# hyperledger-labs/bdls

Measured on AMD Instinct MI355X. Metric: P-256 ECDSA verifies/sec (fused SHA-256, bit-exact vs Go crypto/ecdsa + Fabric low-S), higher is better.
Workload: dtype u32; 1 GPU; BASELINE config 2: 1048576 records/GPU, 256B messages, 65536 distinct keys, 1/16 corrupted, fused SHA-256; records_per_gpu=1048576, records_total=1048576, msg_len=256, nkeys=65536, corrupt_den=16, parallelism=shard1 (no collective)

## Files before the change

### bdls_amd/csrc/bdls_hip.cpp

```cpp
#include <hip/hip_runtime.h>

#include <algorithm>
#include <cctype>
#include <atomic>
#include <chrono>
#include <condition_variable>
#include <deque>
#include <memory>
#include <cstdio>
#include <cstdlib>
#include <cstring>
#include <functional>
#include <mutex>
#include <string>
#include <unordered_map>
#include <thread>
#include <vector>

#include "../../include/bdls_hip.h"
#include "verify.h"
#include "comb384.h"
#include "keys384.h"
#include "verify384.h"
#include "pack.h"
// ... 206 lines not shown
  bool defer = false;
  std::vector<std::vector<hipEvent_t>> ev_pool;
  size_t ev_used = 0;
  const uint32_t* last_counters = nullptr;
  uint32_t last_max_tables = 0, last_wide = 0;
  std::mutex mu;
};

std::mutex g_mu;
std::vector<Dev*> g_devs;

struct LaneRef {
  hipStream_t stream, aux;
  hipEvent_t fork, join, done, build;
  bool* done_recorded;
  DevBuf* ws;
};
LaneRef lane_ref(Dev& d, int l) {
  if (l <= 0) return LaneRef{d.stream, d.aux, d.fork, d.join, d.done, d.build, &d.done_recorded,
                             nullptr};
  Lane1& x = d.xl[l - 1];
  return LaneRef{x.stream, x.aux, x.fork, x.join, x.done, x.build, &x.done_recorded, &x.ws};
}

size_t max_tables_for(size_t ns, bool reg = false) {
  return std::min<size_t>(reg ? ns : ns / 2, size_t(1) << 16);
}

size_t qtab_slots(size_t ns) { return ns <= bh::kWide4Max ? 2 * ns : ns; }

size_t work_bytes(size_t ns) {
  const size_t hc = pow2_at_least(2 * ns);
  const size_t mt = max_tables_for(ns);
  return 4 * 32 * ns + 4 * 36 * ns + ns + qtab_slots(ns) * bh::kQTab * bh::kQPt * 4 +
         bh::kGPartWords * 4 * bh::gpart_slots(ns) +
         hc * (8 + 4 + 4 + 4) + ns * 16 + 16 + mt * 8 + mt * (size_t)bh::kKTabWords * 4 +
         256 * 27;
}

int carve_work(Dev& d, size_t n, bh::Work* w, bh::Plan* pl, bool reg = false,
               DevBuf* ws = nullptr) {
  const size_t ns = round64(n);
  DevBuf& buf = ws ? *ws : d.ws;
  int rc = buf.ensure(work_bytes(ns));
  if (rc) return rc;
  char* p = (char*)buf.p;
  auto take = [&](size_t bytes) {
    char* q = p;
    p += round256(bytes);
    return q;
  };
  w->ns = (uint32_t)ns;
  w->e = (uint32_t*)take(32 * ns);
  w->r = (uint32_t*)take(32 * ns);
  w->sm = (uint32_t*)take(32 * ns);
  w->pre = (uint32_t*)take(32 * ns);
  w->qx = (uint32_t*)take(36 * ns);
  w->qy = (uint32_t*)take(36 * ns);
  w->rm = (uint32_t*)take(36 * ns);
  w->r2m = (uint32_t*)take(36 * ns);
  w->st = (uint8_t*)take(ns);
  w->qtab = (uint32_t*)take(qtab_slots(ns) * bh::kQTab * bh::kQPt * 4);
  w->gpart = (uint32_t*)take(bh::kGPartWords * 4 * bh::gpart_slots(ns));
  const size_t hc = pow2_at_least(2 * ns);
  const size_t mt = max_tables_for(ns, reg);
  pl->hc = (uint32_t)hc;
  pl->max_tables = (uint32_t)mt;
  pl->slot_hash = (uint64_t*)take(hc * 8);
  pl->slot_rep = (uint32_t*)take(hc * 4);
  pl->slot_cnt = (uint32_t*)take(hc * 4);
  pl->slot_tab = (uint32_t*)take(hc * 4);
  pl->rec_slot = (uint32_t*)take(ns * 4);
  pl->comb_list = (uint32_t*)take(ns * 4);
  pl->comb_order = pl->comb_list;
  pl->ladder_list = (uint32_t*)take(ns * 4);
  pl->rec_tab = (uint32_t*)take(ns * 4);
  pl->counters = (uint32_t*)take(16);
  pl->tab_rec = (uint32_t*)take(mt * 4 + 4);
  pl->tab_dst = (uint32_t*)take(mt * 4 + 4);
  pl->tables = (uint32_t*)take(reg ? 4 : mt * (size_t)bh::kKTabWords * 4 + 4);
  return BH_OK;
}

hipError_t wait_lanes(Dev& d, hipStream_t s) {
  hipError_t e = hipSuccess;
  if (d.done_recorded && (e = hipStreamWaitEvent(s, d.done, 0)) != hipSuccess) return e;
  for (Lane1& x : d.xl)
    if (x.done_recorded && s != x.stream && (e = hipStreamWaitEvent(s, x.done, 0)) != hipSuccess)
      return e;
  return e;
}

int sync_lanes(Dev& d) {
// ... 2580 lines not shown
```

### bdls_amd/csrc/curve_consts.h

```cpp
#pragma once
#include <stdint.h>
namespace bh {
struct Fp_p256 {
  static constexpr uint32_t m[8] = {0xffffffffu, 0xffffffffu, 0xffffffffu, 0x00000000u, 0x00000000u, 0x00000000u, 0x00000001u, 0xffffffffu};
  static constexpr uint32_t n0 = 0x00000001u;
  static constexpr uint32_t r1[8] = {0x00000001u, 0x00000000u, 0x00000000u, 0xffffffffu, 0xffffffffu, 0xffffffffu, 0xfffffffeu, 0x00000000u};
  static constexpr uint32_t r2[8] = {0x00000003u, 0x00000000u, 0xffffffffu, 0xfffffffbu, 0xfffffffeu, 0xffffffffu, 0xfffffffdu, 0x00000004u};
  static constexpr uint32_t mm2[8] = {0xfffffffdu, 0xffffffffu, 0xffffffffu, 0x00000000u, 0x00000000u, 0x00000000u, 0x00000001u, 0xffffffffu};
  static constexpr uint32_t r3[8] = {0x0000000au, 0xfffffffdu, 0xfffffff7u, 0xffffffedu, 0xfffffffcu, 0x00000005u, 0x00000001u, 0x00000018u};
  static constexpr int32_t s30[9] = {1073741823, 1073741823, 1073741823, 63, 0, 0, 4096, 1073725440, 65535};
  static constexpr uint32_t inv30 = 0x3fffffffu;
};
struct Fn_p256 {
  static constexpr uint32_t m[8] = {0xfc632551u, 0xf3b9cac2u, 0xa7179e84u, 0xbce6faadu, 0xffffffffu, 0xffffffffu, 0x00000000u, 0xffffffffu};
  static constexpr uint32_t n0 = 0xee00bc4fu;
  static constexpr uint32_t r1[8] = {0x039cdaafu, 0x0c46353du, 0x58e8617bu, 0x43190552u, 0x00000000u, 0x00000000u, 0xffffffffu, 0x00000000u};
  static constexpr uint32_t r2[8] = {0xbe79eea2u, 0x83244c95u, 0x49bd6fa6u, 0x4699799cu, 0x2b6bec59u, 0x2845b239u, 0xf3d95620u, 0x66e12d94u};
  static constexpr uint32_t mm2[8] = {0xfc63254fu, 0xf3b9cac2u, 0xa7179e84u, 0xbce6faadu, 0xffffffffu, 0xffffffffu, 0x00000000u, 0xffffffffu};
  static constexpr uint32_t r3[8] = {0x0b65a624u, 0xac8ebec9u, 0x0c0555c9u, 0x111f28aeu, 0x6ba5e93fu, 0x2543b924u, 0x6407be65u, 0x503a54e7u};
  static constexpr int32_t s30[9] = {1013130577, 250030859, 830072911, 968797033, 1073741756, 1073741823, 4095, 1073725440, 65535};
  static constexpr uint32_t inv30 = 0x11ff43b1u;
};
struct Cv_p256 {
  static constexpr uint32_t b_m[8] = {0x29c4bddfu, 0xd89cdf62u, 0x78843090u, 0xacf005cdu, 0xf7212ed6u, 0xe5a220abu, 0x04874834u, 0xdc30061du};
  static constexpr uint32_t gx_m[8] = {0x18a9143cu, 0x79e730d4u, 0x5fedb601u, 0x75ba95fcu, 0x77622510u, 0x79fb732bu, 0xa53755c6u, 0x18905f76u};
  static constexpr uint32_t gy_m[8] = {0xce95560au, 0xddf25357u, 0xba19e45cu, 0x8b4ab8e4u, 0xdd21f325u, 0xd2e88688u, 0x25885d85u, 0x8571ff18u};
  static constexpr uint32_t half_n[8] = {0x7e3192a8u, 0x79dce561u, 0xd38bcf42u, 0xde737d56u, 0xffffffffu, 0x7fffffffu, 0x80000000u, 0x7fffffffu};
  static constexpr uint32_t p_minus_n[8] = {0x039cdaaeu, 0x0c46353du, 0x58e8617bu, 0x43190553u, 0x00000000u, 0x00000000u, 0x00000000u, 0x00000000u};
  static constexpr uint32_t n[8] = {0xfc632551u, 0xf3b9cac2u, 0xa7179e84u, 0xbce6faadu, 0xffffffffu, 0xffffffffu, 0x00000000u, 0xffffffffu};
  static constexpr uint32_t p[8] = {0xffffffffu, 0xffffffffu, 0xffffffffu, 0x00000000u, 0x00000000u, 0x00000000u, 0x00000001u, 0xffffffffu};
  static constexpr int a_is_minus3 = 1;
};
struct F30_p256 {
  static constexpr uint32_t p[9] = {0x3fffffffu, 0x3fffffffu, 0x3fffffffu, 0x0000003fu, 0x00000000u, 0x00000000u, 0x00001000u, 0x3fffc000u, 0x0000ffffu};
  static constexpr uint32_t n0 = 0x00000001u;
  static constexpr uint32_t r1[9] = {0x00004000u, 0x00000000u, 0x00000000u, 0x3ff00000u, 0x3fffffffu, 0x3fffffffu, 0x3bffffffu, 0x0fffffffu, 0x00000000u};
  static constexpr uint32_t r2[9] = {0x30000000u, 0x00000000u, 0x00000000u, 0x3ffffffcu, 0x3fffffbfu, 0x3fffffbfu, 0x3fffffffu, 0x3ffff7ffu, 0x00004fffu};
  static constexpr uint32_t r3[9] = {0x00006000u, 0x0000a000u, 0x3fff4000u, 0x3fdfffffu, 0x3fb7ffffu, 0x3fcfffffu, 0x3b7fffffu, 0x18ffffffu, 0x00000000u};
  using M32 = Fp_p256;
  static constexpr uint32_t k32[9] = {0x7fffffe0u, 0x7ffffffeu, 0x7ffffffeu, 0x400007feu, 0x3fffffffu, 0x3fffffffu, 0x4001ffffu, 0x7ff7ffffu, 0x001ffffeu};
  static constexpr uint32_t k64[9] = {0x7fffffc0u, 0x7ffffffeu, 0x7ffffffeu, 0x40000ffeu, 0x3fffffffu, 0x3fffffffu, 0x4003ffffu, 0x7fefffffu, 0x003ffffeu};
  static constexpr uint32_t b_m[9] = {0x2f77f70cu, 0x1f6229c4u, 0x02436273u, 0x1cc9c543u, 0x35ab3c01u, 0x2bf7212eu, 0x1025c882u, 0x1e0b7483u, 0x00000187u};
  static constexpr uint32_t gx_m[9] = {0x050f0624u, 0x30d418a9u, 0x1805e79cu, 0x1fc475dbu, 0x041d6ea5u, 0x2b776225u, 0x1985adccu, 0x2bdc755cu, 0x000017ddu};
  static constexpr uint32_t gy_m[9] = {0x1582a15cu, 0x1357ce95u, 0x117377c9u, 0x0e434a9eu, 0x0962d2aeu, 0x08dd21f3u, 0x1535e21au, 0x0aaf85d8u, 0x00007fc6u};
  static constexpr uint32_t pm2[8] = {0xfffffffdu, 0xffffffffu, 0xffffffffu, 0x00000000u, 0x00000000u, 0x00000000u, 0x00000001u, 0xffffffffu};
  static constexpr int a_is_minus3 = 1;
  static constexpr int sparse_p256 = 1;
};
struct Fp_k1 {
  static constexpr uint32_t m[8] = {0xfffffc2fu, 0xfffffffeu, 0xffffffffu, 0xffffffffu, 0xffffffffu, 0xffffffffu, 0xffffffffu, 0xffffffffu};
  static constexpr uint32_t n0 = 0xd2253531u;
  static constexpr uint32_t r1[8] = {0x000003d1u, 0x00000001u, 0x00000000u, 0x00000000u, 0x00000000u, 0x00000000u, 0x00000000u, 0x00000000u};
  static constexpr uint32_t r2[8] = {0x000e90a1u, 0x000007a2u, 0x00000001u, 0x00000000u, 0x00000000u, 0x00000000u, 0x00000000u, 0x00000000u};
  static constexpr uint32_t mm2[8] = {0xfffffc2du, 0xfffffffeu, 0xffffffffu, 0xffffffffu, 0xffffffffu, 0xffffffffu, 0xffffffffu, 0xffffffffu};
  static constexpr uint32_t r3[8] = {0x3795f671u, 0x002bb1e3u, 0x00000b73u, 0x00000001u, 0x00000000u, 0x00000000u, 0x00000000u, 0x00000000u};
  static constexpr int32_t s30[9] = {1073740847, 1073741819, 1073741823, 1073741823, 1073741823, 1073741823, 1073741823, 1073741823, 65535};
  static constexpr uint32_t inv30 = 0x2ddacacfu;
};
struct Fn_k1 {
  static constexpr uint32_t m[8] = {0xd0364141u, 0xbfd25e8cu, 0xaf48a03bu, 0xbaaedce6u, 0xfffffffeu, 0xffffffffu, 0xffffffffu, 0xffffffffu};
  static constexpr uint32_t n0 = 0x5588b13fu;
  static constexpr uint32_t r1[8] = {0x2fc9bebfu, 0x402da173u, 0x50b75fc4u, 0x45512319u, 0x00000001u, 0x00000000u, 0x00000000u, 0x00000000u};
  static constexpr uint32_t r2[8] = {0x67d7d140u, 0x896cf214u, 0x0e7cf878u, 0x741496c2u, 0x5bcd07c6u, 0xe697f5e4u, 0x81c69bc5u, 0x9d671cd5u};
  static constexpr uint32_t mm2[8] = {0xd036413fu, 0xbfd25e8cu, 0xaf48a03bu, 0xbaaedce6u, 0xfffffffeu, 0xffffffffu, 0xffffffffu, 0xffffffffu};
  static constexpr uint32_t r3[8] = {0xe9ff41edu, 0x7bc0cfe0u, 0x44d4322cu, 0x00176484u, 0xf1d0b2dau, 0xb1b31347u, 0x18ef116du, 0x555d800cu};
  static constexpr int32_t s30[9] = {271991105, 1061780019, 881460155, 733428139, 1073741498, 1073741823, 1073741823, 1073741823, 65535};
  static constexpr uint32_t inv30 = 0x2a774ec1u;
};
struct Cv_k1 {
  static constexpr uint32_t b_m[8] = {0x00001ab7u, 0x00000007u, 0x00000000u, 0x00000000u, 0x00000000u, 0x00000000u, 0x00000000u, 0x00000000u};
  static constexpr uint32_t gx_m[8] = {0x487e2097u, 0xd7362e5au, 0x29bc66dbu, 0x231e2953u, 0x33fd129cu, 0x979f48c0u, 0xe9089f48u, 0x9981e643u};
  static constexpr uint32_t gy_m[8] = {0xd3dbabe2u, 0xb15ea6d2u, 0x1f1dc64du, 0x8dfc5d5du, 0xac19c136u, 0x70b6b59au, 0xd4a582d6u, 0xcf3f851fu};
  static constexpr uint32_t half_n[8] = {0x681b20a0u, 0xdfe92f46u, 0x57a4501du, 0x5d576e73u, 0xffffffffu, 0xffffffffu, 0xffffffffu, 0x7fffffffu};
  static constexpr uint32_t p_minus_n[8] = {0x2fc9baeeu, 0x402da172u, 0x50b75fc4u, 0x45512319u, 0x00000001u, 0x00000000u, 0x00000000u, 0x00000000u};
  static constexpr uint32_t n[8] = {0xd0364141u, 0xbfd25e8cu, 0xaf48a03bu, 0xbaaedce6u, 0xfffffffeu, 0xffffffffu, 0xffffffffu, 0xffffffffu};
  static constexpr uint32_t p[8] = {0xfffffc2fu, 0xfffffffeu, 0xffffffffu, 0xffffffffu, 0xffffffffu, 0xffffffffu, 0xffffffffu, 0xffffffffu};
  static constexpr int a_is_minus3 = 0;
};
struct F30_k1 {
  static constexpr uint32_t p[9] = {0x3ffffc2fu, 0x3ffffffbu, 0x3fffffffu, 0x3fffffffu, 0x3fffffffu, 0x3fffffffu, 0x3fffffffu, 0x3fffffffu, 0x0000ffffu};
  static constexpr uint32_t n0 = 0x12253531u;
  static constexpr uint32_t r1[9] = {0x00f44000u, 0x00010000u, 0x00000000u, 0x00000000u, 0x00000000u, 0x00000000u, 0x00000000u, 0x00000000u, 0x00000000u};
  static constexpr uint32_t r2[9] = {0x10000000u, 0x0003a428u, 0x000007a2u, 0x00000004u, 0x00000000u, 0x00000000u, 0x00000000u, 0x00000000u, 0x00000000u};
  static constexpr uint32_t r3[9] = {0x00000000u, 0x1f671000u, 0x2c78cde5u, 0x0b73002bu, 0x00040000u, 0x00000000u, 0x00000000u, 0x00000000u, 0x00000000u};
  using M32 = Fp_k1;
  static constexpr uint32_t k32[9] = {0x7fff85e0u, 0x7fffff7eu, 0x7ffffffeu, 0x7ffffffeu, 0x7ffffffeu, 0x7ffffffeu, 0x7ffffffeu, 0x7ffffffeu, 0x001ffffeu};
  static constexpr uint32_t k64[9] = {0x7fff0bc0u, 0x7ffffefeu, 0x7ffffffeu, 0x7ffffffeu, 0x7ffffffeu, 0x7ffffffeu, 0x7ffffffeu, 0x7ffffffeu, 0x003ffffeu};
  static constexpr uint32_t b_m[9] = {0x06adc000u, 0x00070000u, 0x00000000u, 0x00000000u, 0x00000000u, 0x00000000u, 0x00000000u, 0x00000000u, 0x00000000u};
  static constexpr uint32_t gx_m[9] = {0x08b83460u, 0x2e5ae1feu, 0x1b6f5cd8u, 0x15329bc6u, 0x2708c78au, 0x0033fd12u, 0x225e7d23u, 0x3e9089f4u, 0x00007990u};
  static constexpr uint32_t gy_m[9] = {0x2bbe38ffu, 0x26d3a317u, 0x1936c57au, 0x15d1f1dcu, 0x0da37f17u, 0x1aac19c1u, 0x19c2dad6u, 0x3d4a582du, 0x0000e147u};
  static constexpr uint32_t pm2[8] = {0xfffffc2du, 0xfffffffeu, 0xffffffffu, 0xffffffffu, 0xffffffffu, 0xffffffffu, 0xffffffffu, 0xffffffffu};
  static constexpr int a_is_minus3 = 0;
  static constexpr int sparse_p256 = 0;
};
}
```

### bdls_amd/csrc/fp30.h

```cpp
#pragma once
#include "bh_common.h"
#include "curve_consts.h"

#ifndef BH_ZFILTER
#define BH_ZFILTER 0
#endif

namespace bh {

constexpr uint32_t kM30 = 0x3fffffffu;
constexpr int kL = 9;

BH_HD void f_copy(uint32_t r[9], const uint32_t a[9]) {
#pragma unroll
  for (int i = 0; i < 9; i++) r[i] = a[i];
}

BH_HD void f_sel(uint32_t r[9], bool c, const uint32_t a[9], const uint32_t b[9]) {
#pragma unroll
  for (int i = 0; i < 9; i++) r[i] = c ? a[i] : b[i];
}

template <class C>
BH_HD void f_const(uint32_t r[9], const C& c) {
// ... 27 lines not shown
    }
#pragma unroll
    for (int k = 8; k < 17; k++) {
      acc += C[k];
      const uint32_t m = (uint32_t)acc & kM30;
      if (k == 8) {
        mac_k<64u>(C[11], m);
        mac_k<4096u>(C[14], m);
        mac_k<F::p[7]>(C[15], m);
        mac_k<F::p[8]>(C[16], m);
      } else {
        r[k - 9] = m;
      }
      acc >>= 30;
    }
  } else {
#pragma unroll
    for (int k = 0; k < 17; k++) {
      acc += C[k];
      if (k < 9) {
        const uint32_t m = ((uint32_t)acc * F::n0) & kM30;
        acc += (uint64_t)m * F::p[0];
#pragma unroll
        for (int j = 1; j < 9; j++)
          if (F::p[j]) C[k + j] += (uint64_t)m * F::p[j];
      } else {
        r[k - 9] = (uint32_t)acc & kM30;
      }
      acc >>= 30;
    }
  }
  r[8] = (uint32_t)acc;
}

template <class F>
BH_HD void f_mul(uint32_t r[9], const uint32_t a[9], const uint32_t b[9]) {
  uint64_t C[17];
#pragma unroll
  for (int k = 0; k < 17; k++) C[k] = 0;
#pragma unroll
  for (int i = 0; i < 9; i++)
#pragma unroll
    for (int j = 0; j < 9; j++) C[i + j] += (uint64_t)a[i] * b[j];
  f_redc<F>(r, C);
}

template <class F>
BH_HD void f_sqr(uint32_t r[9], const uint32_t a[9]) {
  uint64_t C[17];
  uint32_t d[9];
#pragma unroll
  for (int i = 0; i < 9; i++) d[i] = a[i] << 1;
#pragma unroll
  for (int k = 0; k < 17; k++) C[k] = 0;
#pragma unroll
  for (int i = 0; i < 9; i++) {
    C[2 * i] += (uint64_t)a[i] * a[i];
#pragma unroll
    for (int j = i + 1; j < 9; j++) C[i + j] += (uint64_t)d[i] * a[j];
  }
  f_redc<F>(r, C);
}

BH_HD void f_add(uint32_t r[9], const uint32_t a[9], const uint32_t b[9]) {
  uint32_t c = 0;
#pragma unroll
// ... 298 lines not shown
```

### bdls_amd/csrc/gen_consts.py

```python
#!/usr/bin/env python3
import sys

CURVES = {
    "p256": dict(
        p=2**256 - 2**224 + 2**192 + 2**96 - 1,
        n=0xFFFFFFFF00000000FFFFFFFFFFFFFFFFBCE6FAADA7179E84F3B9CAC2FC632551,
        a=-3,
        b=0x5AC635D8AA3A93E7B3EBBD55769886BC651D06B0CC53B0F63BCE3C3E27D2604B,
        gx=0x6B17D1F2E12C4247F8BCE6E563A440F277037D812DEB33A0F4A13945D898C296,
        gy=0x4FE342E2FE1A7F9B8EE7EB4A7C0F9E162BCE33576B315ECECBB6406837BF51F5,
    ),
    "k1": dict(
        p=2**256 - 2**32 - 977,
        n=0xFFFFFFFFFFFFFFFFFFFFFFFFFFFFFFFEBAAEDCE6AF48A03BBFD25E8CD0364141,
        a=0,
        b=7,
        gx=0x79BE667EF9DCBBAC55A06295CE870B07029BFCDB2DCE28D959F2815B16F81798,
        gy=0x483ADA7726A3C4655DA4FBFC0E1108A8FD17B448A68554199C47D08FFB10D4B8,
    ),
}
R = 2**256


def limbs(v):
# ... 8 lines not shown
    print(f"  static constexpr uint32_t r1[8] = {{{limbs(R % m)}}};  // R mod m")
    print(f"  static constexpr uint32_t r2[8] = {{{limbs(R * R % m)}}};  // R^2 mod m")
    print(f"  static constexpr uint32_t mm2[8] = {{{limbs(m - 2)}}};  // m - 2 (Fermat exponent)")
    print(f"  static constexpr uint32_t r3[8] = {{{limbs(R * R * R % m)}}};  // R^3 mod m")
    s30 = ", ".join(f"{(m >> (30 * i)) & ((1 << 30) - 1) if i < 8 else m >> 240}" for i in range(9))
    print(f"  static constexpr int32_t s30[9] = {{{s30}}};  // m in signed radix 2^30")
    print(f"  static constexpr uint32_t inv30 = 0x{pow(m, -1, 2**30):08x}u;  // m^-1 mod 2^30")
    print("};")


W = 30
MASK = (1 << W) - 1
R30 = 2**270


def limbs30(v):
    assert 0 <= v < 2**300
    out = [(v >> (W * i)) & MASK for i in range(9)]
    out[8] = v >> (W * 8)
    assert out[8] < 2**32
    return ", ".join(f"0x{x:08x}u" for x in out)


def borrowed30(v):
    l = [(v >> (W * i)) & MASK for i in range(9)]
    l[8] = v >> (W * 8)
    for i in range(8):
        l[i] += 1 << W
        l[i + 1] -= 1
    assert sum(x << (W * i) for i, x in enumerate(l)) == v and min(l) >= 0
    return ", ".join(f"0x{x:08x}u" for x in l)


def emit_fp30(name, c):
    p = c["p"]
    n0 = (-pow(p, -1, 2**W)) % 2**W
    print(f"struct {name} {{  // radix 2^30, R = 2^270")
    print(f"  static constexpr uint32_t p[9] = {{{limbs30(p)}}};")
    print(f"  static constexpr uint32_t n0 = 0x{n0:08x}u;  // -p^-1 mod 2^30")
    print(f"  static constexpr uint32_t r1[9] = {{{limbs30(R30 % p)}}};  // R mod p")
    print(f"  static constexpr uint32_t r2[9] = {{{limbs30(R30 * R30 % p)}}};  // R^2 mod p")
    print(f"  static constexpr uint32_t r3[9] = {{{limbs30(R30 ** 3 % p)}}};  // R^3 mod p (safegcd inverse)")
    print(f"  using M32 = Fp_{name[4:]};  // the same field on 32-bit limbs (fe.h safegcd)")
    print(f"  static constexpr uint32_t k32[9] = {{{borrowed30(32 * p)}}};  // 32p, borrowed form")
    print(f"  static constexpr uint32_t k64[9] = {{{borrowed30(64 * p)}}};  // 64p, borrowed form")
    print(f"  static constexpr uint32_t b_m[9] = {{{limbs30(c['b'] * R30 % p)}}};  // b R mod p")
    print(f"  static constexpr uint32_t gx_m[9] = {{{limbs30(c['gx'] * R30 % p)}}};")
    print(f"  static constexpr uint32_t gy_m[9] = {{{limbs30(c['gy'] * R30 % p)}}};")
    print(f"  static constexpr uint32_t pm2[8] = {{{limbs(p - 2)}}};  // Fermat exponent (32-bit limbs)")
    print(f"  static constexpr int a_is_minus3 = {1 if c['a'] == -3 else 0};")
    print(f"  static constexpr int sparse_p256 = {1 if p == 2**256 - 2**224 + 2**192 + 2**96 - 1 else 0};")
    print("};")


def main():
    print("// GENERATED by gen_consts.py -- do not edit.")
    print("#pragma once")
    print("#include <stdint.h>")
    print("namespace bh {")
    for cname, c in CURVES.items():
        emit_mod(f"Fp_{cname}", c["p"])
        emit_mod(f"Fn_{cname}", c["n"])
        p = c["p"]
        print(f"struct Cv_{cname} {{")
        print(f"  static constexpr uint32_t b_m[8] = {{{limbs(c['b'] * R % p)}}};  // b*R mod p")
        print(f"  static constexpr uint32_t gx_m[8] = {{{limbs(c['gx'] * R % p)}}};")
        print(f"  static constexpr uint32_t gy_m[8] = {{{limbs(c['gy'] * R % p)}}};")
        print(f"  static constexpr uint32_t half_n[8] = {{{limbs(c['n'] >> 1)}}};  // floor(n/2)")
        print(f"  static constexpr uint32_t p_minus_n[8] = {{{limbs(p - c['n'])}}};  // p - n")
        print(f"  static constexpr uint32_t n[8] = {{{limbs(c['n'])}}};")
        print(f"  static constexpr uint32_t p[8] = {{{limbs(p)}}};")
        print(f"  static constexpr int a_is_minus3 = {1 if c['a'] == -3 else 0};")
        print("};")
        emit_fp30(f"F30_{cname}", c)
    print("}  // namespace bh")


P384 = dict(
    p=2**384 - 2**128 - 2**96 + 2**32 - 1,
    n=0xFFFFFFFFFFFFFFFFFFFFFFFFFFFFFFFFFFFFFFFFFFFFFFFFC7634D81F4372DDF581A0DB248B0A77AECEC196ACCC52973,
    a=-3,
    b=0xB3312FA7E23EE7E4988E056BE3F82D19181D9C6EFE8141120314088F5013875AC656398D8A2ED19D2A85C8EDD3EC2AEF,
    gx=0xAA87CA22BE8B05378EB1C71EF320AD746E1D3B628BA79B9859F741E082542A385502F25DBF55296C3A545E3872760AB7,
    gy=0x3617DE4A96262C6F5D9E98BF9292DC29F8F41DBD289A147CE9DA3113B5F0B8C00A60B1CE1D7E819D7A431D7C90EA0E5F,
)
W28 = 28
L28 = 14
R28 = 2**(W28 * L28)
KP_MAX = 32


def limbs28(v):
    assert 0 <= v < R28
    return ", ".join(f"0x{(v >> (W28 * i)) & (2**W28 - 1):07x}u" for i in range(L28))


def words12(v):
    assert 0 <= v < 2**384
    return ", ".join(f"0x{(v >> (32 * i)) & 0xffffffff:08x}u" for i in range(12))


def emit_mod28(name, m):
    n0 = (-pow(m, -1, 2**W28)) % 2**W28
    print(f"struct {name} {{  // radix 2^28, 14 limbs, R = 2^392")
    print(f"  static constexpr uint32_t m[14] = {{{limbs28(m)}}};")
    print(f"  static constexpr uint32_t n0 = 0x{n0:07x}u;  // -m^-1 mod 2^28")
# ... 35 lines not shown
```

### bdls_amd/csrc/verify.h

```cpp
#pragma once
#include <type_traits>

#include "blake2b.h"
#include "der.h"
#include "fe.h"
#include "ec30.h"
#include "sha256.h"
#include "sha3.h"

namespace bh {

enum : uint32_t {
  BHF_HASH_SHA256 = 1u,
  BHF_NO_LOW_S = 2u,
  BHF_HASH_SHA3_256 = 8u,
  BHF_BDLS_PREHASHED = 0x100u,
};

enum : int { HK_GIVEN_OR_SHA256 = 0, HK_SHA3_256 = 1 };

enum : uint8_t { ST_R2OK = 0x80u };

struct BatchIn {
  const uint8_t* pub;
// ... 97 lines not shown
};

#ifndef BH_AOS
#define BH_AOS 1
#endif
BH_HD void ld8(uint32_t v[8], const uint32_t* base, uint32_t i, uint32_t ns) {
#if BH_AOS
  const W4* p = reinterpret_cast<const W4*>(base + (size_t)i * 8);
  const W4 a = p[0], b = p[1];
  v[0] = a.x; v[1] = a.y; v[2] = a.z; v[3] = a.w;
  v[4] = b.x; v[5] = b.y; v[6] = b.z; v[7] = b.w;
#else
#pragma unroll
  for (int k = 0; k < 8; k++) v[k] = base[(size_t)k * ns + i];
#endif
}
BH_HD void st8(uint32_t* base, uint32_t i, uint32_t ns, const uint32_t v[8]) {
#if BH_AOS
  W4* p = reinterpret_cast<W4*>(base + (size_t)i * 8);
  p[0] = W4{v[0], v[1], v[2], v[3]};
  p[1] = W4{v[4], v[5], v[6], v[7]};
#else
#pragma unroll
  for (int k = 0; k < 8; k++) base[(size_t)k * ns + i] = v[k];
#endif
}
BH_HD void ld9(uint32_t v[9], const uint32_t* base, uint32_t i, uint32_t ns) {
#pragma unroll
  for (int k = 0; k < 9; k++) v[k] = BH_AOS ? base[(size_t)i * 9 + k] : base[(size_t)k * ns + i];
}
BH_HD void st9(uint32_t* base, uint32_t i, uint32_t ns, const uint32_t v[9]) {
#pragma unroll
  for (int k = 0; k < 9; k++) (BH_AOS ? base[(size_t)i * 9 + k] : base[(size_t)k * ns + i]) = v[k];
}

template <class P, class C>
BH_HD bool key_import(const uint8_t* q, uint32_t qx30[9], uint32_t qy30[9]) {
  uint32_t qx[8], qy[8], pp[8];
  load_const8(pp, C::p);
  be32_to_limbs(qx, q);
  be32_to_limbs(qy, q + 32);
  if (geq8(qx, pp) || geq8(qy, pp)) return false;
  f_from_u256(qx30, qx);
  f_from_u256(qy30, qy);
  f_to_mont<P>(qx30, qx30);
  f_to_mont<P>(qy30, qy30);
  f_canon<P>(qx30, qx30);
  f_canon<P>(qy30, qy30);
  return j_on_curve<P>(qx30, qy30);
}

template <class P, class C>
BH_HD void stage_prep_key(const BatchIn& in, const Work& w, uint32_t i) {
  uint32_t qx30[9], qy30[9];
  const bool ok = key_import<P, C>(in.pub + (size_t)i * 64, qx30, qy30);
  if (!ok) {
    f_const(qx30, P::gx_m);
    f_const(qy30, P::gy_m);
  }
  st9(w.qx, i, w.ns, qx30);
  st9(w.qy, i, w.ns, qy30);
  w.st[i] = ok ? (uint8_t)R_OK : (uint8_t)R_BAD_KEY;
}

template <class C, int HK>
BH_HD void digest_e(const BatchIn& in, uint32_t i, uint32_t e[8]) {
// ... 26 lines not shown
  uint32_t nn[8], t[8];
  load_const8(nn, C::n);
  const uint32_t bo = sub8(t, e, nn);
  if (!bo) copy8(e, t);
}

template <class P, class N, class C, int HK = HK_GIVEN_OR_SHA256, bool DEFER = false>
BH_HD void stage_prep(const BatchIn& in, const Work& w, uint32_t i) {
  uint8_t reason = R_OK;
  uint32_t r[8], s[8], e[8];
  uint32_t qx30[9], qy30[9];
  const uint32_t slen = in.sig_len[i];
  const uint32_t mlen = in.msg_len[i];
  const bool fused = HK == HK_SHA3_256 || (in.flags & BHF_HASH_SHA256) != 0;
  if (slen == 0) reason = R_EMPTY_SIG;
  else if (!fused && mlen == 0) reason = R_EMPTY_DIGEST;
  DerSig ds;
  if (reason == R_OK) reason = der_parse_sig(in.sig + in.sig_off[i], slen, &ds);
  uint32_t half[8], nn[8];
  load_const8(half, C::half_n);
  load_const8(nn, C::n);
  if (reason == R_OK) {
    copy8(r, ds.r);
    copy8(s, ds.s);
    if (!(in.flags & BHF_NO_LOW_S) && (ds.s_big || !geq8(half, s))) reason = R_HIGH_S;
  }
  if (reason == R_OK && !key_import<P, C>(in.pub + (size_t)i * 64, qx30, qy30))
    reason = R_BAD_KEY;
  if (reason == R_OK && (ds.r_big || geq8(r, nn))) reason = R_R_RANGE;
  if (reason == R_OK && (ds.s_big || geq8(s, nn))) reason = R_S_RANGE;
  if (reason == R_OK && !DEFER) digest_e<C, HK>(in, i, e);
  uint8_t st = reason;
  if (reason == R_OK) {
    uint32_t pmn[8], rn[8], rm[9], r2m[9];
    load_const8(pmn, C::p_minus_n);
    f_from_u256(rm, r);
    f_to_mont<P>(rm, rm);
    f_canon<P>(rm, rm);
    if (!geq8(r, pmn)) {
      st |= ST_R2OK;
      add8(rn, r, nn);
      f_from_u256(r2m, rn);
      f_to_mont<P>(r2m, r2m);
      f_canon<P>(r2m, r2m);
    } else {
      f_copy(r2m, rm);
    }
    st9(w.rm, i, w.ns, rm);
    st9(w.r2m, i, w.ns, r2m);
    to_mont<N>(s, s);
  } else {
    for (int k = 0; k < 8; k++) { e[k] = r[k] = 0; }
    e[0] = r[0] = 1;
    load_const8(s, N::r1);
    f_const(qx30, P::gx_m);
    f_const(qy30, P::gy_m);
  }
  if (!DEFER) st8(w.e, i, w.ns, e);
  st8(w.r, i, w.ns, r);
  st8(w.sm, i, w.ns, s);
  st9(w.qx, i, w.ns, qx30);
  st9(w.qy, i, w.ns, qy30);
  w.st[i] = st;
}

BH_HD void setbytes_u256(const uint8_t* b, uint32_t len, uint32_t v[8], bool* big, bool* zero) {
  uint32_t lo = 0;
  while (lo < len && b[lo] == 0) lo++;
  const uint32_t L = len - lo;
  *zero = (L == 0);
  *big = (L > 32);
#pragma unroll
  for (int k = 0; k < 8; k++) v[k] = 0;
  if (L > 32) return;
#pragma unroll
  for (int j = 0; j < 32; j++) {
    uint32_t x = 0;
    if ((uint32_t)j < L) x = b[len - 1 - j];
    v[j >> 2] |= x << (8 * (j & 3));
  }
}

template <class C>
BH_HD void stage_bdls_given(const BdlsIn& in, const Work& w, uint32_t i) {
  uint32_t e[8], nn[8], t[8];
  const uint8_t* m = in.msg + in.msg_off[i];
  const uint32_t mlen = in.msg_len[i];
// ... 13 lines not shown

template <class C>
BH_HD void stage_bdls_hash(const BdlsIn& in, const Work& w, uint32_t i) {
  if (in.flags & BHF_BDLS_PREHASHED) return stage_bdls_given<C>(in, w, i);
  uint8_t hsh[32];
  uint32_t e[8], nn[8], t[8];
  const uint8_t* q = in.xy + (size_t)i * 64;
  bdls_signed_proto_hash(hsh, in.version[i], q, q + 32, in.msg + in.msg_off[i], in.msg_len[i]);
  be32_to_limbs(e, hsh);
  load_const8(nn, C::n);
  if (!sub8(t, e, nn)) copy8(e, t);
  st8(w.e, i, w.ns, e);
}

template <class P, class N, class C>
BH_HD void stage_prep(const BdlsIn& in, const Work& w, uint32_t i) {
  uint8_t reason = R_OK;
  uint32_t r[8], s[8], nn[8];
  uint32_t qx30[9], qy30[9];
  load_const8(nn, C::n);
  bool rbig, rzero, sbig, szero;
  setbytes_u256(in.r + in.r_off[i], in.r_len[i], r, &rbig, &rzero);
  setbytes_u256(in.s + in.s_off[i], in.s_len[i], s, &sbig, &szero);
  if (rzero) reason = R_R_NONPOS;
  else if (szero) reason = R_S_NONPOS;
  const uint8_t* q = in.xy + (size_t)i * 64;
  const bool badkey = reason == R_OK && !key_import<P, C>(q, qx30, qy30);
  if (badkey && P::a_is_minus3) reason = R_BAD_KEY;
  if (reason == R_OK && (rbig || geq8(r, nn))) reason = R_R_RANGE;
  if (reason == R_OK && (sbig || geq8(s, nn))) reason = R_S_RANGE;
  if (reason == R_OK && badkey) reason = R_MATH;
  uint8_t st = reason;
  if (reason == R_OK) {
    uint32_t pmn[8], rn[8], rm[9], r2m[9];
    load_const8(pmn, C::p_minus_n);
    f_from_u256(rm, r);
    f_to_mont<P>(rm, rm);
    f_canon<P>(rm, rm);
    if (!geq8(r, pmn)) {
      st |= ST_R2OK;
      add8(rn, r, nn);
      f_from_u256(r2m, rn);
      f_to_mont<P>(r2m, r2m);
      f_canon<P>(r2m, r2m);
    } else {
      f_copy(r2m, rm);
    }
    st9(w.rm, i, w.ns, rm);
    st9(w.r2m, i, w.ns, r2m);
    to_mont<N>(s, s);
  } else {
    for (int k = 0; k < 8; k++) r[k] = 0;
    r[0] = 1;
    load_const8(s, N::r1);
    f_const(qx30, P::gx_m);
    f_const(qy30, P::gy_m);
  }
  st8(w.r, i, w.ns, r);
  st8(w.sm, i, w.ns, s);
  st9(w.qx, i, w.ns, qx30);
  st9(w.qy, i, w.ns, qy30);
  w.st[i] = st;
}

template <class N, bool U1 = true, bool VAR = false>
BH_HD void stage_inv(const Work& w, uint32_t c, uint32_t stride, uint32_t n) {
  uint32_t acc[8], x[8];
  load_const8(acc, N::r1);
  uint32_t last = c;
  for (uint32_t i = c; i < n; i += stride) {
    st8(w.pre, i, w.ns, acc);
    ld8(x, w.sm, i, w.ns);
    mont_mul<N>(acc, acc, x);
    last = i;
  }
  if (c >= n) return;
  uint32_t inv[8];
  mont_inv_sg<N, VAR>(inv, acc);
  for (uint32_t i = last;; i -= stride) {
    uint32_t pre[8], wi[8], t[8];
    ld8(pre, w.pre, i, w.ns);
    mont_mul<N>(wi, inv, pre);
    ld8(x, w.sm, i, w.ns);
    mont_mul<N>(inv, inv, x);
    if constexpr (U1) {
      ld8(t, w.e, i, w.ns);
      mont_mul<N>(t, t, wi);
      st8(w.e, i, w.ns, t);
    } else {
      st8(w.sm, i, w.ns, wi);
    }
    ld8(t, w.r, i, w.ns);
    mont_mul<N>(t, t, wi);
    st8(w.r, i, w.ns, t);
    if (i < c + stride) break;
  }
}

template <class N>
BH_HD void calc_u1(uint32_t u1[8], const Work& w, uint32_t i) {
  uint32_t wi[8];
  ld8(u1, w.e, i, w.ns);
  ld8(wi, w.sm, i, w.ns);
  mont_mul<N>(u1, u1, wi);
}

BH_HD void booth5(uint32_t in6, uint32_t* mag, bool* neg) {
  uint32_t sgn = 0u - (in6 >> 5);
  uint32_t d = (63u - in6) & sgn;
  d |= in6 & ~sgn;
  *mag = (d >> 1) + (d & 1u);
  *neg = sgn != 0;
}


BH_HD uint32_t* qtab_entry(uint32_t* tab, uint32_t wave, uint32_t entry, uint32_t lane) {
  return tab + (((size_t)wave * 64 + lane) * kQTab + entry) * kQPt;
}

BH_HD void qtab_store(uint32_t* tab, uint32_t wave, uint32_t entry, uint32_t lane, const J30& P) {
  uint32_t v[28];
#pragma unroll
  for (int k = 0; k < 9; k++) {
    v[k] = P.X[k];
    v[9 + k] = P.Y[k];
    v[18 + k] = P.Z[k];
  }
  v[27] = 0;
  W4* d = reinterpret_cast<W4*>(qtab_entry(tab, wave, entry, lane));
#pragma unroll
  for (int q = 0; q < 7; q++) d[q] = W4{v[4 * q], v[4 * q + 1], v[4 * q + 2], v[4 * q + 3]};
}

BH_HD void qtab_load(J30& P, const uint32_t* tab, uint32_t wave, uint32_t entry, uint32_t lane) {
  const W4* s = reinterpret_cast<const W4*>(qtab_entry(const_cast<uint32_t*>(tab), wave, entry, lane));
  uint32_t v[28];
#pragma unroll
// ... 155 lines not shown
      mag = nmag;
      neg = nneg;
    } else {
      g_window(v, win, gtab, tx, ty, mag, neg);
      if (neg) f_neg<P, 64>(ty, ty);
      g_step<P>(B, b_inf, tx, ty, mag, one);
    }
  }
}

template <class P>
BH_HD bool finish_check(const Work& w, uint32_t i, const J30& A, bool a_inf, const J30& B,
                        bool b_inf) {
  J30 Pt;
  bool p_inf;
  if (b_inf) {
    j_copy(Pt, A);
    p_inf = a_inf;
  } else if (a_inf) {
    j_copy(Pt, B);
    p_inf = false;
  } else {
    bool same;
    const bool deg = j_add<P>(Pt, A, B, &same);
    p_inf = false;
    if (deg) {
      if (same) j_dbl<P>(Pt, A);
      else p_inf = true;
    }
  }
  uint32_t z2[9], t[9], x[9], rm[9];
  f_sqr<P>(z2, Pt.Z);
  const bool z_zero = f_is_zero2<P>(z2);
  f_reduce<P>(x, Pt.X);
  ld9(rm, w.rm, i, w.ns);
  f_mul<P>(t, rm, z2);
  f_canon<P>(t, t);
  bool ok = f_eq(t, x);
  if (w.st[i] & ST_R2OK) {
    ld9(rm, w.r2m, i, w.ns);
    f_mul<P>(t, rm, z2);
    f_canon<P>(t, t);
    ok = ok || f_eq(t, x);
  }
  return ok && !p_inf && !z_zero;
}

template <class P>
BH_HD void q_ladder(J30& A, bool& a_inf, const Work& w, uint32_t i, uint32_t wave,
                    uint32_t lane) {
  uint32_t u2[8], qx[9], qy[9], one[9];
  ld8(u2, w.r, i, w.ns);
  ld9(qx, w.qx, i, w.ns);
  ld9(qy, w.qy, i, w.ns);
  f_const(one, P::r1);
  J30 T;
  f_copy(T.X, qx);
  f_copy(T.Y, qy);
  f_copy(T.Z, one);
  qtab_store(w.qtab, wave, 0, lane, T);
  j_dbl<P>(T, T);
  qtab_store(w.qtab, wave, 1, lane, T);
  for (uint32_t k = 2; k < kQTab; k++) {
    bool same;
    j_madd<P>(T, T, qx, qy, &same);
    qtab_store(w.qtab, wave, k, lane, T);
  }
  uint32_t K[9];
  K[0] = u2[0] << 28;
#pragma unroll
  for (int k = 1; k < 8; k++) K[k] = (u2[k] << 28) | (u2[k - 1] >> 4);
  K[8] = u2[7] >> 4;
  {
    uint32_t mag;
    bool neg;
    booth5(K[8] >> 26, &mag, &neg);
// ... 1360 lines not shown
```

Before: 209.3 million verifies/s.

## Move scalar arithmetic onto the radix-2^30 multiplier and drop stored r+n candidate

```diff
diff --git a/bdls_amd/csrc/bdls_hip.cpp b/bdls_amd/csrc/bdls_hip.cpp
--- a/bdls_amd/csrc/bdls_hip.cpp
+++ b/bdls_amd/csrc/bdls_hip.cpp
@@ -262,7 +262,7 @@
 size_t work_bytes(size_t ns) {
   const size_t hc = pow2_at_least(2 * ns);
   const size_t mt = max_tables_for(ns);
-  return 4 * 32 * ns + 4 * 36 * ns + ns + qtab_slots(ns) * bh::kQTab * bh::kQPt * 4 +
+  return 4 * 32 * ns + 3 * 36 * ns + ns + qtab_slots(ns) * bh::kQTab * bh::kQPt * 4 +
          bh::kGPartWords * 4 * bh::gpart_slots(ns) +
          hc * (8 + 4 + 4 + 4) + ns * 16 + 16 + mt * 8 + mt * (size_t)bh::kKTabWords * 4 +
          256 * 27;
@@ -288,7 +288,7 @@
   w->qx = (uint32_t*)take(36 * ns);
   w->qy = (uint32_t*)take(36 * ns);
   w->rm = (uint32_t*)take(36 * ns);
-  w->r2m = (uint32_t*)take(36 * ns);
+  w->r2m = nullptr;
   w->st = (uint8_t*)take(ns);
   w->qtab = (uint32_t*)take(qtab_slots(ns) * bh::kQTab * bh::kQPt * 4);
   w->gpart = (uint32_t*)take(bh::kGPartWords * 4 * bh::gpart_slots(ns));
diff --git a/bdls_amd/csrc/curve_consts.h b/bdls_amd/csrc/curve_consts.h
--- a/bdls_amd/csrc/curve_consts.h
+++ b/bdls_amd/csrc/curve_consts.h
@@ -1,6 +1,7 @@
 #pragma once
 #include <stdint.h>
 namespace bh {
+template <class M> struct Scalar30;
 struct Fp_p256 {
   static constexpr uint32_t m[8] = {0xffffffffu, 0xffffffffu, 0xffffffffu, 0x00000000u, 0x00000000u, 0x00000000u, 0x00000001u, 0xffffffffu};
   static constexpr uint32_t n0 = 0x00000001u;
@@ -31,6 +32,16 @@
   static constexpr uint32_t p[8] = {0xffffffffu, 0xffffffffu, 0xffffffffu, 0x00000000u, 0x00000000u, 0x00000000u, 0x00000001u, 0xffffffffu};
   static constexpr int a_is_minus3 = 1;
 };
+struct N30_p256 {
+  static constexpr uint32_t p[9] = {0x3c632551u, 0x0ee72b0bu, 0x3179e84fu, 0x39beab69u, 0x3fffffbcu, 0x3fffffffu, 0x00000fffu, 0x3fffc000u, 0x0000ffffu};
+  static constexpr uint32_t n0 = 0x2e00bc4fu;
+  static constexpr uint32_t r1[9] = {0x36abc000u, 0x353d039cu, 0x05ec3118u, 0x15258e86u, 0x0010c641u, 0x00000000u, 0x3c000000u, 0x0fffffffu, 0x00000000u};
+  static constexpr uint32_t r2[9] = {0x0887ac57u, 0x05d911a5u, 0x130785e0u, 0x2a328ab8u, 0x19076a9eu, 0x1afb1658u, 0x2484a92bu, 0x2a0ebf05u, 0x000055abu};
+  static constexpr uint32_t r3[9] = {0x2fc38adfu, 0x3fa3e2bbu, 0x1b018b23u, 0x095feb0bu, 0x110fb41du, 0x13f26264u, 0x0f2dd97au, 0x0c894964u, 0x0000084du};
+  using M32 = Fn_p256;
+  static constexpr int sparse_p256 = 0;
+};
+template <> struct Scalar30<Fn_p256> { using type = N30_p256; };
 struct F30_p256 {
   static constexpr uint32_t p[9] = {0x3fffffffu, 0x3fffffffu, 0x3fffffffu, 0x0000003fu, 0x00000000u, 0x00000000u, 0x00001000u, 0x3fffc000u, 0x0000ffffu};
   static constexpr uint32_t n0 = 0x00000001u;
@@ -38,6 +49,7 @@
   static constexpr uint32_t r2[9] = {0x30000000u, 0x00000000u, 0x00000000u, 0x3ffffffcu, 0x3fffffbfu, 0x3fffffbfu, 0x3fffffffu, 0x3ffff7ffu, 0x00004fffu};
   static constexpr uint32_t r3[9] = {0x00006000u, 0x0000a000u, 0x3fff4000u, 0x3fdfffffu, 0x3fb7ffffu, 0x3fcfffffu, 0x3b7fffffu, 0x18ffffffu, 0x00000000u};
   using M32 = Fp_p256;
+  using N30 = N30_p256;
   static constexpr uint32_t k32[9] = {0x7fffffe0u, 0x7ffffffeu, 0x7ffffffeu, 0x400007feu, 0x3fffffffu, 0x3fffffffu, 0x4001ffffu, 0x7ff7ffffu, 0x001ffffeu};
   static constexpr uint32_t k64[9] = {0x7fffffc0u, 0x7ffffffeu, 0x7ffffffeu, 0x40000ffeu, 0x3fffffffu, 0x3fffffffu, 0x4003ffffu, 0x7fefffffu, 0x003ffffeu};
   static constexpr uint32_t b_m[9] = {0x2f77f70cu, 0x1f6229c4u, 0x02436273u, 0x1cc9c543u, 0x35ab3c01u, 0x2bf7212eu, 0x1025c882u, 0x1e0b7483u, 0x00000187u};
@@ -77,6 +89,16 @@
   static constexpr uint32_t p[8] = {0xfffffc2fu, 0xfffffffeu, 0xffffffffu, 0xffffffffu, 0xffffffffu, 0xffffffffu, 0xffffffffu, 0xffffffffu};
   static constexpr int a_is_minus3 = 0;
 };
+struct N30_k1 {
+  static constexpr uint32_t p[9] = {0x10364141u, 0x3f497a33u, 0x348a03bbu, 0x2bb739abu, 0x3ffffebau, 0x3fffffffu, 0x3fffffffu, 0x3fffffffu, 0x0000ffffu};
+  static constexpr uint32_t n0 = 0x1588b13fu;
+  static constexpr uint32_t r1[9] = {0x2fafc000u, 0x21732fc9u, 0x3f1100b6u, 0x31950b75u, 0x00515448u, 0x00000000u, 0x00000000u, 0x00000000u, 0x00000000u};
+  static constexpr uint32_t r2[9] = {0x3c6a0df3u, 0x090ea30du, 0x103606edu, 0x17c0c584u, 0x01a618aeu, 0x3341f1cfu, 0x17f5e45bu, 0x1a6f179au, 0x0000581cu};
+  static constexpr uint32_t r3[9] = {0x18c893ddu, 0x32d33b61u, 0x27b6f6f1u, 0x0d469a63u, 0x19757685u, 0x2da6c922u, 0x11fc742cu, 0x2db1b313u, 0x0000bc45u};
+  using M32 = Fn_k1;
+  static constexpr int sparse_p256 = 0;
+};
+template <> struct Scalar30<Fn_k1> { using type = N30_k1; };
 struct F30_k1 {
   static constexpr uint32_t p[9] = {0x3ffffc2fu, 0x3ffffffbu, 0x3fffffffu, 0x3fffffffu, 0x3fffffffu, 0x3fffffffu, 0x3fffffffu, 0x3fffffffu, 0x0000ffffu};
   static constexpr uint32_t n0 = 0x12253531u;
@@ -84,6 +106,7 @@
   static constexpr uint32_t r2[9] = {0x10000000u, 0x0003a428u, 0x000007a2u, 0x00000004u, 0x00000000u, 0x00000000u, 0x00000000u, 0x00000000u, 0x00000000u};
   static constexpr uint32_t r3[9] = {0x00000000u, 0x1f671000u, 0x2c78cde5u, 0x0b73002bu, 0x00040000u, 0x00000000u, 0x00000000u, 0x00000000u, 0x00000000u};
   using M32 = Fp_k1;
+  using N30 = N30_k1;
   static constexpr uint32_t k32[9] = {0x7fff85e0u, 0x7fffff7eu, 0x7ffffffeu, 0x7ffffffeu, 0x7ffffffeu, 0x7ffffffeu, 0x7ffffffeu, 0x7ffffffeu, 0x001ffffeu};
   static constexpr uint32_t k64[9] = {0x7fff0bc0u, 0x7ffffefeu, 0x7ffffffeu, 0x7ffffffeu, 0x7ffffffeu, 0x7ffffffeu, 0x7ffffffeu, 0x7ffffffeu, 0x003ffffeu};
   static constexpr uint32_t b_m[9] = {0x06adc000u, 0x00070000u, 0x00000000u, 0x00000000u, 0x00000000u, 0x00000000u, 0x00000000u, 0x00000000u, 0x00000000u};
diff --git a/bdls_amd/csrc/fp30.h b/bdls_amd/csrc/fp30.h
--- a/bdls_amd/csrc/fp30.h
+++ b/bdls_amd/csrc/fp30.h
@@ -83,6 +83,24 @@
   }
   r[8] = (uint32_t)acc;
 }
+
+template <class F>
+constexpr bool redc_generic_fits(uint64_t top) {
+  unsigned __int128 carry = 0;
+  for (int k = 0; k < 17; k++) {
+    unsigned __int128 col = carry;
+    for (int i = 0; i < 9; i++) {
+      const int j = k - i;
+      if (j < 0 || j > 8) continue;
+      col += (unsigned __int128)(i < 8 ? kM30 : top) * (j < 8 ? kM30 : top);
+      col += (unsigned __int128)kM30 * F::p[j];
+    }
+    if (col >> 64) return false;
+    carry = col >> 30;
+  }
+  return (carry >> 32) == 0;
+}
+constexpr uint64_t kScalarTop = 1u << 18;
 
 template <class F>
 BH_HD void f_mul(uint32_t r[9], const uint32_t a[9], const uint32_t b[9]) {
diff --git a/bdls_amd/csrc/gen_consts.py b/bdls_amd/csrc/gen_consts.py
--- a/bdls_amd/csrc/gen_consts.py
+++ b/bdls_amd/csrc/gen_consts.py
@@ -64,6 +64,20 @@
     return ", ".join(f"0x{x:08x}u" for x in l)
 
 
+def emit_n30(cname, n):
+    n0 = (-pow(n, -1, 2**W)) % 2**W
+    print(f"struct N30_{cname} {{  // group order n, radix 2^30, R = 2^270")
+    print(f"  static constexpr uint32_t p[9] = {{{limbs30(n)}}};  // n (the modulus of f_redc / f_canon)")
+    print(f"  static constexpr uint32_t n0 = 0x{n0:08x}u;  // -n^-1 mod 2^30")
+    print(f"  static constexpr uint32_t r1[9] = {{{limbs30(R30 % n)}}};  // R mod n")
+    print(f"  static constexpr uint32_t r2[9] = {{{limbs30(R30 * R30 % n)}}};  // R^2 mod n")
+    print(f"  static constexpr uint32_t r3[9] = {{{limbs30(R30 ** 3 % n)}}};  // R^3 mod n (safegcd inverse)")
+    print(f"  using M32 = Fn_{cname};  // the same modulus on 32-bit limbs (fe.h safegcd)")
+    print("  static constexpr int sparse_p256 = 0;")
+    print("};")
+    print(f"template <> struct Scalar30<Fn_{cname}> {{ using type = N30_{cname}; }};")
+
+
 def emit_fp30(name, c):
     p = c["p"]
     n0 = (-pow(p, -1, 2**W)) % 2**W
@@ -74,6 +88,7 @@
     print(f"  static constexpr uint32_t r2[9] = {{{limbs30(R30 * R30 % p)}}};  // R^2 mod p")
     print(f"  static constexpr uint32_t r3[9] = {{{limbs30(R30 ** 3 % p)}}};  // R^3 mod p (safegcd inverse)")
     print(f"  using M32 = Fp_{name[4:]};  // the same field on 32-bit limbs (fe.h safegcd)")
+    print(f"  using N30 = N30_{name[4:]};  // the curve's group order on the same multiplier")
     print(f"  static constexpr uint32_t k32[9] = {{{borrowed30(32 * p)}}};  // 32p, borrowed form")
     print(f"  static constexpr uint32_t k64[9] = {{{borrowed30(64 * p)}}};  // 64p, borrowed form")
     print(f"  static constexpr uint32_t b_m[9] = {{{limbs30(c['b'] * R30 % p)}}};  // b R mod p")
@@ -90,6 +105,7 @@
     print("#pragma once")
     print("#include <stdint.h>")
     print("namespace bh {")
+    print("template <class M> struct Scalar30;  // Fn_* -> its radix-2^30 class")
     for cname, c in CURVES.items():
         emit_mod(f"Fp_{cname}", c["p"])
         emit_mod(f"Fn_{cname}", c["n"])
@@ -104,6 +120,7 @@
         print(f"  static constexpr uint32_t p[8] = {{{limbs(p)}}};")
         print(f"  static constexpr int a_is_minus3 = {1 if c['a'] == -3 else 0};")
         print("};")
+        emit_n30(cname, c["n"])
         emit_fp30(f"F30_{cname}", c)
     print("}  // namespace bh")
 
diff --git a/bdls_amd/csrc/verify.h b/bdls_amd/csrc/verify.h
--- a/bdls_amd/csrc/verify.h
+++ b/bdls_amd/csrc/verify.h
@@ -153,6 +153,46 @@
 BH_HD void st9(uint32_t* base, uint32_t i, uint32_t ns, const uint32_t v[9]) {
 #pragma unroll
   for (int k = 0; k < 9; k++) (BH_AOS ? base[(size_t)i * 9 + k] : base[(size_t)k * ns + i]) = v[k];
+}
+
+template <class N>
+using S30 = typename Scalar30<N>::type;
+
+template <class N>
+BH_HD void n_mul(uint32_t r[9], const uint32_t a[9], const uint32_t b[9]) {
+  static_assert(redc_generic_fits<S30<N>>(kScalarTop), "scalar f_redc column bound");
+  f_mul<S30<N>>(r, a, b);
+}
+BH_HD void n_ld(uint32_t v[9], const uint32_t* base, uint32_t i, uint32_t ns) {
+  uint32_t x[8];
+  ld8(x, base, i, ns);
+  f_from_u256(v, x);
+}
+template <class N>
+BH_HD void n_words(uint32_t r[8], const uint32_t a[9]) {
+  uint32_t c[9];
+  f_canon<S30<N>>(c, a);
+  f_to_u256(r, c);
+}
+template <class N>
+BH_HD void n_st(uint32_t* base, uint32_t i, uint32_t ns, const uint32_t a[9]) {
+  uint32_t x[8];
+  n_words<N>(x, a);
+  st8(base, i, ns, x);
+}
+template <class N>
+BH_HD void n_to_mont(uint32_t r[8], const uint32_t a[8]) {
+  uint32_t t[9], r2[9];
+  f_from_u256(t, a);
+  f_const(r2, S30<N>::r2);
+  n_mul<N>(t, t, r2);
+  n_words<N>(r, t);
+}
+template <class N>
+BH_HD void n_one_mont(uint32_t r[8]) {
+  uint32_t t[9];
+  f_const(t, S30<N>::r1);
+  f_to_u256(r, t);
 }
 
 template <class P, class C>
@@ -245,27 +285,16 @@
   if (reason == R_OK && !DEFER) digest_e<C, HK>(in, i, e);
   uint8_t st = reason;
   if (reason == R_OK) {
-    uint32_t pmn[8], rn[8], rm[9], r2m[9];
+    uint32_t pmn[8], rm[9];
     load_const8(pmn, C::p_minus_n);
     f_from_u256(rm, r);
-    f_to_mont<P>(rm, rm);
-    f_canon<P>(rm, rm);
-    if (!geq8(r, pmn)) {
-      st |= ST_R2OK;
-      add8(rn, r, nn);
-      f_from_u256(r2m, rn);
-      f_to_mont<P>(r2m, r2m);
-      f_canon<P>(r2m, r2m);
-    } else {
-      f_copy(r2m, rm);
-    }
+    if (!geq8(r, pmn)) st |= ST_R2OK;
     st9(w.rm, i, w.ns, rm);
-    st9(w.r2m, i, w.ns, r2m);
-    to_mont<N>(s, s);
+    n_to_mont<N>(s, s);
   } else {
     for (int k = 0; k < 8; k++) { e[k] = r[k] = 0; }
     e[0] = r[0] = 1;
-    load_const8(s, N::r1);
+    n_one_mont<N>(s);
     f_const(qx30, P::gx_m);
     f_const(qy30, P::gy_m);
   }
@@ -345,27 +374,16 @@
   if (reason == R_OK && badkey) reason = R_MATH;
   uint8_t st = reason;
   if (reason == R_OK) {
-    uint32_t pmn[8], rn[8], rm[9], r2m[9];
+    uint32_t pmn[8], rm[9];
     load_const8(pmn, C::p_minus_n);
     f_from_u256(rm, r);
-    f_to_mont<P>(rm, rm);
-    f_canon<P>(rm, rm);
-    if (!geq8(r, pmn)) {
-      st |= ST_R2OK;
-      add8(rn, r, nn);
-      f_from_u256(r2m, rn);
-      f_to_mont<P>(r2m, r2m);
-      f_canon<P>(r2m, r2m);
-    } else {
-      f_copy(r2m, rm);
-    }
+    if (!geq8(r, pmn)) st |= ST_R2OK;
     st9(w.rm, i, w.ns, rm);
-    st9(w.r2m, i, w.ns, r2m);
-    to_mont<N>(s, s);
+    n_to_mont<N>(s, s);
   } else {
     for (int k = 0; k < 8; k++) r[k] = 0;
     r[0] = 1;
-    load_const8(s, N::r1);
+    n_one_mont<N>(s);
     f_const(qx30, P::gx_m);
     f_const(qy30, P::gy_m);
   }
@@ -378,44 +396,49 @@
 
 template <class N, bool U1 = true, bool VAR = false>
 BH_HD void stage_inv(const Work& w, uint32_t c, uint32_t stride, uint32_t n) {
-  uint32_t acc[8], x[8];
-  load_const8(acc, N::r1);
+  uint32_t acc[9], x[9];
+  f_const(acc, S30<N>::r1);
   uint32_t last = c;
   for (uint32_t i = c; i < n; i += stride) {
-    st8(w.pre, i, w.ns, acc);
-    ld8(x, w.sm, i, w.ns);
-    mont_mul<N>(acc, acc, x);
+    n_st<N>(w.pre, i, w.ns, acc);
+    n_ld(x, w.sm, i, w.ns);
+    n_mul<N>(acc, acc, x);
     last = i;
   }
   if (c >= n) return;
-  uint32_t inv[8];
-  mont_inv_sg<N, VAR>(inv, acc);
+  uint32_t inv[9], a8[8], r3[9];
+  n_words<N>(a8, acc);
+  mod_inv_sg<N, VAR>(a8, a8);
+  f_from_u256(inv, a8);
+  f_const(r3, S30<N>::r3);
+  n_mul<N>(inv, inv, r3);
   for (uint32_t i = last;; i -= stride) {
-    uint32_t pre[8], wi[8], t[8];
-    ld8(pre, w.pre, i, w.ns);
-    mont_mul<N>(wi, inv, pre);
-    ld8(x, w.sm, i, w.ns);
-    mont_mul<N>(inv, inv, x);
+    uint32_t pre[9], wi[9], t[9];
+    n_ld(pre, w.pre, i, w.ns);
+    n_mul<N>(wi, inv, pre);
+    n_ld(x, w.sm, i, w.ns);
+    n_mul<N>(inv, inv, x);
     if constexpr (U1) {
-      ld8(t, w.e, i, w.ns);
-      mont_mul<N>(t, t, wi);
-      st8(w.e, i, w.ns, t);
+      n_ld(t, w.e, i, w.ns);
+      n_mul<N>(t, t, wi);
+      n_st<N>(w.e, i, w.ns, t);
     } else {
-      st8(w.sm, i, w.ns, wi);
-    }
-    ld8(t, w.r, i, w.ns);
-    mont_mul<N>(t, t, wi);
-    st8(w.r, i, w.ns, t);
+      n_st<N>(w.sm, i, w.ns, wi);
+    }
+    n_ld(t, w.r, i, w.ns);
+    n_mul<N>(t, t, wi);
+    n_st<N>(w.r, i, w.ns, t);
     if (i < c + stride) break;
   }
 }
 
 template <class N>
 BH_HD void calc_u1(uint32_t u1[8], const Work& w, uint32_t i) {
-  uint32_t wi[8];
-  ld8(u1, w.e, i, w.ns);
-  ld8(wi, w.sm, i, w.ns);
-  mont_mul<N>(u1, u1, wi);
+  uint32_t e[9], wi[9];
+  n_ld(e, w.e, i, w.ns);
+  n_ld(wi, w.sm, i, w.ns);
+  n_mul<N>(e, e, wi);
+  n_words<N>(u1, e);
 }
 
 BH_HD void booth5(uint32_t in6, uint32_t* mag, bool* neg) {
@@ -637,16 +660,20 @@
   uint32_t z2[9], t[9], x[9], rm[9];
   f_sqr<P>(z2, Pt.Z);
   const bool z_zero = f_is_zero2<P>(z2);
-  f_reduce<P>(x, Pt.X);
+  const uint32_t one[9] = {1, 0, 0, 0, 0, 0, 0, 0, 0};
+  f_mul<P>(x, Pt.X, one);
+  f_canon<P>(x, x);
   ld9(rm, w.rm, i, w.ns);
-  f_mul<P>(t, rm, z2);
-  f_canon<P>(t, t);
-  bool ok = f_eq(t, x);
-  if (w.st[i] & ST_R2OK) {
-    ld9(rm, w.r2m, i, w.ns);
+  bool ok = false;
+  const int cands = (w.st[i] & ST_R2OK) ? 2 : 1;
+#pragma unroll 1
+  for (int c = 0; c < cands; c++) {
     f_mul<P>(t, rm, z2);
     f_canon<P>(t, t);
     ok = ok || f_eq(t, x);
+    uint32_t nn[9];
+    f_const(nn, P::N30::p);
+    f_add(rm, rm, nn);
   }
   return ok && !p_inf && !z_zero;
 }
```

New measurement: 209.8 million verifies/s, median of 5. No clear change (+0.2%).
